# sirpkt/flink-tensorflow

Hardware: AMD Instinct MI355X
Metric: records/sec (whole node) + p50 per-record latency, ResNet-50 stream DP=1/8 (higher is better)
Workload: dtype bf16

## Files before the change

### flink_tensorflow_amd/kernels/conv_pp.hip

```cpp
#include <pybind11/pybind11.h>

#include <stdexcept>
#include <string>
#include <type_traits>

#include "common.h"

namespace {


struct CSrc {
  const bf16* x;
  int H, W, C;
  int sh, sw, ph, pw;
};

struct CPParams {
  CSrc s[2];
  const bf16* w;
  const float* bias;
  const bf16* res;
  void* y;
  int M, N, K;
  int OH, OW;
  int KW, dh, dw;
  int ldw, ldy, y_coff, ldr;
  int tiles_m, tiles_n;
  int nk0;
};

FTM_DEVICE int lite_slot(int row, int chunk) { return chunk ^ (row & 7); }

template <int ACT, bool HAS_RES, bool DUAL = false>
__global__ __launch_bounds__(256, 2) void conv_lite_kernel(CPParams p) {
  constexpr int BM = 128, BN = 128, BK = 64;
  constexpr int NT = 256;
  constexpr int ROWB = BK * 2;
  constexpr int RPI = 1024 / ROWB;
  constexpr int Q = 4;
  constexpr int NI = BN / 32;
  constexpr int PJ = 4;
  constexpr int XB = BM * ROWB, WB = BN * ROWB, STG = XB + WB;
  constexpr int OPITCH = BN * 2 + 16;
  constexpr int LDS = 2 * STG;
  static_assert(BM / RPI / 4 == Q && BN / RPI / 4 == Q && BM * OPITCH <= LDS, "tile geometry");
  __shared__ __attribute__((aligned(1024))) uint8_t smem[LDS];

  const int nwg = p.tiles_m * p.tiles_n;
  const int tile = xcd_remap(blockIdx.x, nwg);
  const int tm = tile / p.tiles_n;
  const int tn = tile - tm * p.tiles_n;
  const int m0 = tm * BM;
  const int n0 = tn * BN;
  const int lane = threadIdx.x & 63;
  const int wave = __builtin_amdgcn_readfirstlane(threadIdx.x >> 6);
  const int wm = wave & 1;
  const int wn = wave >> 1;

  const int drow = lane / 8;
  const int dchunk = lite_slot(drow, lane % 8);
  const unsigned nimg = (unsigned)p.M / (unsigned)(p.OH * p.OW);
  const CSrc& S = p.s[0];
  const __amdgpu_buffer_rsrc_t rx = __builtin_amdgcn_make_buffer_rsrc(
      (void*)S.x, 0, (int)(nimg * (unsigned)(S.H * S.W) * (unsigned)S.C * 2u), 0x00020000);
  const __amdgpu_buffer_rsrc_t rw = __builtin_amdgcn_make_buffer_rsrc(
      (void*)p.w, 0, (int)((unsigned)p.N * (unsigned)p.ldw * 2u), 0x00020000);
  int pb[4], hw[4], pb1[4];
  unsigned offw[4];
  const CSrc& S1 = p.s[1];
  __amdgpu_buffer_rsrc_t rx1 = rx;
  if constexpr (DUAL)
    rx1 = __builtin_amdgcn_make_buffer_rsrc((void*)S1.x, 0, (int)(nimg * (unsigned)(S1.H * S1.W) * (unsigned)S1.C * 2u),
                                            0x00020000);
  const int ohw = p.OH * p.OW;
#pragma unroll
  for (int q = 0; q < Q; ++q) {
    const unsigned co = n0 + RPI * (Q * wave + q) + drow;
    offw[q] = co < (unsigned)p.N ? (co * p.ldw + dchunk * 8) * 2u : 0x80000000u;
    const int r = RPI * (Q * wave + q) + drow;
    const int m = m0 + r;
    const bool live = m < p.M;
    const int n = live ? m / ohw : 0;
    const int rem = live ? m - n * ohw : 0;
    const int oh = rem / p.OW;
    const int ow = rem - oh * p.OW;
    const int ih0 = live ? oh * S.sh - S.ph : -16384;
    const int iw0 = ow * S.sw - S.pw;
    pb[q] = ((n * S.H + ih0) * S.W + iw0) * S.C * 2 + dchunk * 16;
    hw[q] = (ih0 << 16) | (iw0 & 0xFFFF);
    if constexpr (DUAL) pb1[q] = live ? ((n * S1.H + oh * S1.sh) * S1.W + ow * S1.sw) * S1.C * 2 + dchunk * 16 : -1;
  }
  const int cpt = S.C / BK;
  int cc = 0, kw = 0, kh = 0, kt_dma = 0;
  auto dma = [&](int stage) {
    const unsigned woff = (unsigned)kt_dma * (unsigned)ROWB;
    if constexpr (DUAL) {
      if (kt_dma >= p.nk0) {
        const int delta1 = (kt_dma - p.nk0) * BK * 2;
        ++kt_dma;
        uint8_t* bx = smem + stage * STG + Q * wave * RPI * ROWB;
        uint8_t* bw = smem + stage * STG + XB + Q * wave * RPI * ROWB;
#pragma unroll
        for (int q = 0; q < Q; ++q) {
          __builtin_amdgcn_raw_ptr_buffer_load_lds(rx1, (__attribute__((address_space(3))) void*)(bx + q * 1024), 16,
                                                   pb1[q] >= 0 ? (unsigned)(pb1[q] + delta1) : 0x80000000u, 0, 0, 0);
          __builtin_amdgcn_raw_ptr_buffer_load_lds(rw, (__attribute__((address_space(3))) void*)(bw + q * 1024), 16,
                                                   offw[q], woff, 0, 0);
        }
        return;
      }
    }
    const int dih = kh * p.dh, diw = kw * p.dw;
    const int delta = ((dih * S.W + diw) * S.C + cc * BK) * 2;
    ++kt_dma;
    if (++cc == cpt) {
      cc = 0;
      if (++kw == p.KW) {
        kw = 0;
        ++kh;
      }
    }
    uint8_t* bx = smem + stage * STG + Q * wave * RPI * ROWB;
    uint8_t* bw = smem + stage * STG + XB + Q * wave * RPI * ROWB;
#pragma unroll
    for (int q = 0; q < Q; ++q) {
      const int ih = (hw[q] >> 16) + dih;
      const int iw = ((hw[q] << 16) >> 16) + diw;
      const bool ok = (unsigned)ih < (unsigned)S.H && (unsigned)iw < (unsigned)S.W;
      __builtin_amdgcn_raw_ptr_buffer_load_lds(rx, (__attribute__((address_space(3))) void*)(bx + q * 1024), 16,
                                               ok ? (unsigned)(pb[q] + delta) : 0x80000000u, 0, 0, 0);
      __builtin_amdgcn_raw_ptr_buffer_load_lds(rw, (__attribute__((address_space(3))) void*)(bw + q * 1024), 16,
                                               offw[q], woff, 0, 0);
    }
  };

  const int frow = lane & 15;
  const int fq = lane >> 4;
  f32x4 acc[NI][PJ];
#pragma unroll
  for (int i = 0; i < NI; ++i)
#pragma unroll
    for (int j = 0; j < PJ; ++j) acc[i][j] = f32x4{0.f, 0.f, 0.f, 0.f};

  const int nk = p.K / BK;
  dma(0);
  for (int kt = 0; kt < nk; ++kt) {
    const int st = kt & 1;
    asm volatile("s_waitcnt vmcnt(0)" ::: "memory");
    __syncthreads();
    if (kt + 1 < nk) dma(st ^ 1);
    const uint8_t* xs = smem + st * STG;
    const uint8_t* ws = xs + XB;
    __builtin_amdgcn_s_setprio(1);
#pragma unroll
    for (int ks = 0; ks < BK / 32; ++ks) {
      const int sl = lite_slot(frow, ks * 4 + fq) << 4;
      bf16x8 a[NI], b[PJ];
#pragma unroll
      for (int i = 0; i < NI; ++i)
        a[i] = *reinterpret_cast<const bf16x8*>(ws + (wn * (BN / 2) + i * 16 + frow) * ROWB + sl);
#pragma unroll
      for (int j = 0; j < PJ; ++j) b[j] = *reinterpret_cast<const bf16x8*>(xs + (wm * 64 + j * 16 + frow) * ROWB + sl);
#pragma unroll
      for (int i = 0; i < NI; ++i)
#pragma unroll
        for (int j = 0; j < PJ; ++j) acc[i][j] = __builtin_amdgcn_mfma_f32_16x16x32_bf16(a[i], b[j], acc[i][j], 0, 0, 0);
    }
    __builtin_amdgcn_s_setprio(0);
  }
  __syncthreads();

#pragma unroll
  for (int i = 0; i < NI; ++i) {
    const int cl = wn * (BN / 2) + i * 16 + fq * 4;
    f32x4 bv = {0.f, 0.f, 0.f, 0.f};
    if (p.bias && n0 + cl < p.N) bv = *reinterpret_cast<const f32x4*>(p.bias + n0 + cl);
#pragma unroll
    for (int j = 0; j < PJ; ++j) {
      const int pl = wm * 64 + j * 16 + frow;
      bf16x4 o;
#pragma unroll
      for (int r = 0; r < 4; ++r) {
        float v = acc[i][j][r] + bv[r];
        if constexpr (!HAS_RES) v = apply_act<ACT>(v);
        o[r] = f2bf(v);
      }
      *reinterpret_cast<bf16x4*>(smem + pl * OPITCH + cl * 2) = o;
    }
  }
  __syncthreads();
  bf16* y = reinterpret_cast<bf16*>(p.y);
  constexpr int SEGS = BN / 8;
#pragma unroll 4
  for (int q = threadIdx.x; q < BM * SEGS; q += NT) {
    const int ml = q / SEGS;
    const int ccol = q - ml * SEGS;
    const int m = m0 + ml;
    const int n = n0 + ccol * 8;
    if (m >= p.M || n >= p.N) continue;
    u32x4 v = *reinterpret_cast<const u32x4*>(smem + ml * OPITCH + ccol * 16);
    if constexpr (HAS_RES) {
      bf16x8 o = __builtin_bit_cast(bf16x8, v);
      const bf16x8 r = *reinterpret_cast<const bf16x8*>(p.res + (size_t)m * p.ldr + n);
#pragma unroll
      for (int e = 0; e < 8; ++e) o[e] = f2bf(apply_act<ACT>((float)o[e] + (float)r[e]));
      v = __builtin_bit_cast(u32x4, o);
    }
    *reinterpret_cast<u32x4*>(y + (size_t)m * p.ldy + p.y_coff + n) = v;
  }
}

template <int ACT>
void launch_lite(const CPParams& p, hipStream_t s, bool dual) {
  const dim3 grid(p.tiles_m * p.tiles_n), block(256);
  if (dual) {
    if (p.res) hipLaunchKernelGGL((conv_lite_kernel<ACT, true, true>), grid, block, 0, s, p);
    else hipLaunchKernelGGL((conv_lite_kernel<ACT, false, true>), grid, block, 0, s, p);
    return;
  }
  if (p.res) hipLaunchKernelGGL((conv_lite_kernel<ACT, true>), grid, block, 0, s, p);
  else hipLaunchKernelGGL((conv_lite_kernel<ACT, false>), grid, block, 0, s, p);
}

void need(bool ok, const char* what) {
  if (!ok) throw std::invalid_argument(std::string("conv_pp: ") + what);
}

}

void conv_pp(pybind11::list srcs, uintptr_t w, uintptr_t bias, uintptr_t res, uintptr_t y, int N, int OH, int OW,
             int Cout, int ldy, int y_coff, int ldr, int act, uintptr_t stream) {
  const int ns = (int)pybind11::len(srcs);
  need(ns == 1 || ns == 2, "one or two sources");
  CPParams p{};
  long K = 0;
  for (int i = 0; i < ns; ++i) {
    pybind11::tuple t = srcs[i].cast<pybind11::tuple>();
    need(t.size() == 13, "source tuple (x, N, H, W, C, KH, KW, sh, sw, ph, pw, dh, dw)");
    CSrc& S = p.s[i];
    S.x = reinterpret_cast<const bf16*>(t[0].cast<uintptr_t>());
    const int n = t[1].cast<int>();
    S.H = t[2].cast<int>(); S.W = t[3].cast<int>(); S.C = t[4].cast<int>();
    const int KH = t[5].cast<int>(), KW = t[6].cast<int>();
    S.sh = t[7].cast<int>(); S.sw = t[8].cast<int>(); S.ph = t[9].cast<int>(); S.pw = t[10].cast<int>();
    const int dh = t[11].cast<int>(), dw = t[12].cast<int>();
    need(n == N, "source batch != output batch");
    need(S.C % 64 == 0, "input channels must be a multiple of 64");
    need(reinterpret_cast<uintptr_t>(S.x) % 16 == 0, "x alignment");
    need((long)N * S.H * S.W * S.C * 2 < (1L << 31), "input larger than 2 GiB");
    need(S.H < 16384 && S.W < 16384 && S.ph < 1024 && S.pw < 1024, "spatial size");
    need((KH - 1) * dh < 1024 && (KW - 1) * dw < 1024, "receptive field");
    K += (long)KH * KW * S.C;
    if (i == 0) {
      p.KW = KW;
      p.dh = dh;
      p.dw = dw;
      p.nk0 = (int)(K / 64);
    } else {
      need(KH == 1 && KW == 1 && S.ph == 0 && S.pw == 0, "the 4-wave tile's second source must be 1x1 unpadded");
      need((OH - 1) * S.sh < S.H && (OW - 1) * S.sw < S.W, "second source smaller than the output grid");
    }
  }
  for (int i = ns; i < 2; ++i) p.s[i] = p.s[0];
  need(Cout % 8 == 0 && ldy % 8 == 0 && y_coff % 8 == 0, "Cout / ldy / y_coff must be multiples of 8");
  need(!res || ldr % 8 == 0, "ldr alignment");
  need(w % 16 == 0 && y % 16 == 0 && (!bias || bias % 16 == 0) && (!res || res % 16 == 0), "alignment");
  need((long)Cout * K * 2 < (1L << 31), "weights larger than 2 GiB");
  p.w = reinterpret_cast<const bf16*>(w);
  p.bias = reinterpret_cast<const float*>(bias);
  p.res = reinterpret_cast<const bf16*>(res);
  p.y = reinterpret_cast<void*>(y);
  p.M = N * OH * OW;
  p.N = Cout;
  p.K = (int)K;
  p.OH = OH; p.OW = OW;
  p.ldw = (int)K; p.ldy = ldy; p.y_coff = y_coff; p.ldr = ldr;
  p.tiles_m = (p.M + 127) / 128;
  p.tiles_n = (Cout + 127) / 128;
  hipStream_t s = reinterpret_cast<hipStream_t>(stream);
  if (act == ACT_RELU) launch_lite<ACT_RELU>(p, s, ns == 2);
  else if (act == ACT_NONE) launch_lite<ACT_NONE>(p, s, ns == 2);
  else throw std::invalid_argument("conv_pp: unsupported activation");
  FTM_CHECK_LAUNCH();
}

void register_conv_pp(pybind11::module_& m) {
  m.def("conv_pp", &conv_pp);
}
```

### flink_tensorflow_amd/ops/kernels.py

```python
from __future__ import annotations

import copy
import functools
import math
import os

import torch
import torch.nn.functional as F

from .. import _ext

ACT_NONE, ACT_RELU, ACT_GELU, ACT_SIGMOID, ACT_TANH, ACT_RELU6, ACT_DRELU = 0, 1, 2, 3, 4, 5, 6
_ACT_NAMES = {None: ACT_NONE, "none": ACT_NONE, "relu": ACT_RELU, "gelu": ACT_GELU, "gelu_tanh": ACT_GELU,
              "sigmoid": ACT_SIGMOID, "tanh": ACT_TANH, "relu6": ACT_RELU6, "drelu": ACT_DRELU}


def act_code(act) -> int:
    if isinstance(act, int):
        return act
    try:
        return _ACT_NAMES[act]
    except KeyError:
        raise ValueError(f"unknown activation {act!r}") from None

# ... 182 lines not shown
    if tuple(w3.reshape(w3.shape[0], -1).shape) != (co, k3) or tuple(w1.reshape(cn, -1).shape) != (cn, co):
        raise ValueError(f"bottleneck_tail: weights must be [{co}, {k3}] and [{cn}, {co}], got {tuple(w3.shape)} "
                         f"{tuple(w1.shape)}")
    if b3.numel() != co or b1.numel() != cn:
        raise ValueError("bottleneck_tail: bias sizes must match the output channels")
    odt = x2.dtype if x2.is_cuda else torch.float32
    lead3 = (lead[0], dec_hw[0] // 2, dec_hw[1] // 2) if y3_decimated else lead
    y3 = torch.empty((*lead3, co), dtype=odt, device=x2.device) if y3 is None else y3
    y1 = torch.empty((*lead, cn), dtype=odt, device=x2.device) if y1 is None else y1
    if tuple(y3.shape) != (*lead3, co) or tuple(y1.shape) != (*lead, cn):
        raise ValueError("bottleneck_tail: output buffers do not fit")
    M = x2.numel() // cx
    second = xs if dual else res
    if x2.is_cuda:
        for t, n in ((x2, "x2"), (second, "xs" if dual else "res"), (w3, "w3"), (w1, "w1"), (y3, "y3"), (y1, "y1")):
            _check(t, n, device=x2.device)
        _check(b3, "b3", torch.float32, x2.device)
        _check(b1, "b1", torch.float32, x2.device)
        dev = x2.device.index if x2.device.index is not None else torch.cuda.current_device()
        _hip().bottleneck_tail_bf16(x2.data_ptr(), _ptr(xs), _ptr(res), w3.data_ptr(), b3.data_ptr(),
                                    w1.data_ptr(), b1.data_ptr(), y3.data_ptr(), y1.data_ptr(), M, cn,
                                    _NUM_CU[dev], _stream(), dec_hw[0], dec_hw[1])
        return y3, y1
    xin = torch.cat([x2.reshape(M, cx), xs.reshape(M, cx)], 1) if dual else x2.reshape(M, cx)
    a = xin.float() @ w3.reshape(co, k3).float().t() + b3.float()
    a = a.to(odt).float()
    a = torch.relu(a if dual else a + res.reshape(M, co).float()).to(y3.dtype)
    y3.copy_(a.reshape(*lead, co)[:, ::2, ::2] if y3_decimated else a.reshape(y3.shape))
    b = torch.relu(a.float() @ w1.reshape(cn, co).float().t() + b1.float())
    y1.copy_(b.reshape(y1.shape).to(y1.dtype))
    return y3, y1


def bottleneck_chain(links, w1: torch.Tensor, b1: torch.Tensor, y1: torch.Tensor | None = None,
                     y3: torch.Tensor | None = None, y3_decimated: bool = False, store_y3: bool = True):
    x0 = links[0][0]
    lead = x0.shape[:-1]
    M = x0.numel() // 64
    cn = w1.shape[0]
    if not 1 <= len(links) <= 3 or links[0][1] is None or any(l[1] is not None for l in links[1:]):
        raise ValueError("bottleneck_chain: 1 to 3 links, the first dual ([x | xs]), the others plain")
    for j, (x, xs, w, b) in enumerate(links):
        if x.shape[-1] != 64 or x.numel() != M * 64 or (xs is not None and tuple(xs.shape) != tuple(x.shape)):
            raise ValueError("bottleneck_chain: every source is [..., 64] over the same pixels")
        if tuple(w.reshape(w.shape[0], -1).shape) != (256, 128 if j == 0 else 64) or b.numel() != 256:
            raise ValueError(f"bottleneck_chain: link {j} weights must be [256, {128 if j == 0 else 64}]")
    if cn not in (64, 128) or tuple(w1.reshape(cn, -1).shape) != (cn, 256) or b1.numel() != cn:
        raise ValueError("bottleneck_chain: w1 must be [64 or 128, 256]")
    dec_hw = (0, 0)
    if y3_decimated:
        if x0.dim() != 4 or x0.shape[1] % 2 or x0.shape[2] % 2:
            raise ValueError("bottleneck_chain: decimated y3 needs [N, H, W, 64] sources with even H, W")
        dec_hw = (x0.shape[1], x0.shape[2])
    odt = x0.dtype if x0.is_cuda else torch.float32
    lead3 = (lead[0], dec_hw[0] // 2, dec_hw[1] // 2) if y3_decimated else lead
    if store_y3 and y3 is None:
        y3 = torch.empty((*lead3, 256), dtype=odt, device=x0.device)
    y1 = torch.empty((*lead, cn), dtype=odt, device=x0.device) if y1 is None else y1
    if (store_y3 and tuple(y3.shape) != (*lead3, 256)) or tuple(y1.shape) != (*lead, cn):
        raise ValueError("bottleneck_chain: output buffers do not fit")
    if x0.is_cuda:
        for j, (x, xs, w, b) in enumerate(links):
            for t, n in ((x, "x"), (w, "w")) + (((xs, "xs"),) if xs is not None else ()):
                _check(t, f"link {j} {n}", device=x0.device)
            _check(b, f"link {j} bias", torch.float32, x0.device)
        _check(w1, "w1", device=x0.device)
        _check(b1, "b1", torch.float32, x0.device)
        _check(y1, "y1", device=x0.device)
        if store_y3:
            _check(y3, "y3", device=x0.device)
        dev = x0.device.index if x0.device.index is not None else torch.cuda.current_device()
        _hip().bottleneck_chain_bf16([(x.data_ptr(), _ptr(xs), w.data_ptr(), b.data_ptr()) for x, xs, w, b in links],
                                     w1.data_ptr(), b1.data_ptr(), y3.data_ptr() if store_y3 else 0, y1.data_ptr(), M,
                                     cn, _NUM_CU[dev], _stream(), dec_hw[0], dec_hw[1])
        return (y3 if store_y3 else None), y1
    y = None
    rdt = y1.dtype
    for x, xs, w, b in links:
        xin = torch.cat([x.reshape(M, 64), xs.reshape(M, 64)], 1) if xs is not None else x.reshape(M, 64)
        a = (xin.float() @ w.reshape(256, -1).float().t() + b.float()).to(odt).float()
        y = torch.relu(a if y is None else a + y).to(rdt).float()
    if store_y3:
        y3.copy_(y.reshape(*lead, 256)[:, ::2, ::2] if y3_decimated else y.reshape(y3.shape))
    y1.copy_(torch.relu(y @ w1.reshape(cn, 256).float().t() + b1.float()).reshape(y1.shape).to(y1.dtype))
    return (y3 if store_y3 else None), y1


def gemm(x: torch.Tensor, w_nk: torch.Tensor, bias: torch.Tensor | None = None, residual: torch.Tensor | None = None,
         act=None, out: torch.Tensor | None = None, cfg: int = -1) -> torch.Tensor:
    a = act_code(act)
    lead = x.shape[:-1]
    K = x.shape[-1]
    N, K2 = w_nk.shape
    if K != K2:
        raise ValueError(f"gemm: K mismatch {K} vs {K2}")
    x2 = x.reshape(-1, K)
    M = x2.shape[0]
    if out is None:
        out = torch.empty((*lead, N), dtype=x.dtype if x.is_cuda else torch.float32, device=x.device)
    out2 = out.reshape(M, N)
    if residual is not None and residual.numel() != M * N:
        raise ValueError("gemm: residual shape mismatch")
    if x.is_cuda:
        _check(x2, "x", device=x.device)
        _check(w_nk, "w", device=x.device)
        _check(out2, "out", device=x.device)
        if bias is not None:
            _check(bias, "bias", torch.float32, x.device)
        else:
            bias = _zeros_bias(N, x.device)
        if residual is not None:
            _check(residual, "residual", device=x.device)
        _hip().gemm_bf16(x2.data_ptr(), w_nk.data_ptr(), bias.data_ptr(), _ptr(residual), out2.data_ptr(), M, N, K, K,
                         N, N, a, _stream(), cfg)
        return out
    y = x2.float() @ w_nk.float().t()
    if bias is not None:
        y = y + bias.float()
    if residual is not None:
        y = y + residual.reshape(M, N).float()
    out2.copy_(_apply_act_ref(y, a).to(out.dtype))
    return out


_TR_KTILE_US = 0.45
_TR_KTILE_DEEP_US = 0.3
_TR_SLOTS = 512


def _tr_time(tiles: int, per: int, se: int, num_cu: int = 256) -> float:
    wgs = tiles * se
    if wgs <= num_cu:
        return per * _TR_KTILE_DEEP_US
    return -(-wgs // _TR_SLOTS) * per * _TR_KTILE_US


def gemm_train_splits(M: int, N: int, K: int) -> int:
    tiles = -(-M // 128) * -(-N // 128)
    nk = -(-K // 64)
    best_s, best_t = 1, _tr_time(tiles, nk, 1)
    for s in (2, 3, 4, 6, 8, 12, 16, 24, 32):
        if s > nk:
            break
        per = -(-nk // s)
        se = -(-nk // per)
        t = _tr_time(tiles, per, se) + se * M * N * 8 / _PP_SPLIT_BW + 2.0
        if t < 0.9 * best_t:
            best_s, best_t = se, t
    return best_s


def gemm_train(x: torch.Tensor, w: torch.Tensor, *, x_t: bool = False, w_t: bool = False,
               bias: torch.Tensor | None = None, mask: torch.Tensor | None = None, act=None,
               out: torch.Tensor | None = None, out_dtype=torch.bfloat16, splits: int | None = None,
               ws: torch.Tensor | None = None, colsum: torch.Tensor | None = None) -> torch.Tensor:
    a = act_code(act)
    if mask is not None:
        if a not in (ACT_NONE, ACT_DRELU):
            raise ValueError("gemm_train: mask is the ReLU-backward operand; it takes no other activation")
        a = ACT_DRELU
    M, K = (x.shape[1], x.shape[0]) if x_t else (x.shape[0], x.shape[1])
    N, K2 = (w.shape[1], w.shape[0]) if w_t else (w.shape[0], w.shape[1])
    if K != K2:
        raise ValueError(f"gemm_train: K mismatch {K} vs {K2}")
    if out is None:
        out = torch.empty((M, N), dtype=out_dtype, device=x.device)
    if tuple(out.shape) != (M, N):
        raise ValueError(f"gemm_train: out shape {tuple(out.shape)} != {(M, N)}")
    f32 = out.dtype == torch.float32
    if not x.is_cuda:
        X = x.float().t() if x_t else x.float()
        W = w.float() if w_t else w.float().t()
        y = X @ W
        if bias is not None:
            y = y + bias.float()
        if mask is not None:
            y = torch.where(mask.float() > 0, y, torch.zeros_like(y))
        else:
            y = _apply_act_ref(y, a)
        out.copy_(y.to(out.dtype))
        if colsum is not None:
            yq = out.float()
            for t in range(colsum.shape[0]):
                colsum[t].copy_(yq[t * 128:(t + 1) * 128].sum(0))
        return out
    for t, nm in ((x, "x"), (w, "w")):
        if t.dtype != torch.bfloat16 or t.device != x.device or t.dim() != 2 or t.stride(1) != 1:
            raise ValueError(f"gemm_train: {nm} must be a bf16 [rows, cols] view with contiguous rows on {x.device}")
    if out.stride(1) != 1:
        raise ValueError("gemm_train: out rows must be contiguous")
    if bias is not None:
        _check(bias, "bias", torch.float32, x.device)
    if mask is not None:
        if mask.dtype != torch.bfloat16 or mask.device != x.device:
            raise ValueError(f"gemm_train: mask must be bf16 on {x.device}")
        if tuple(mask.shape) != (M, N) or mask.stride(1) != 1:
            raise ValueError("gemm_train: mask must be [M, N] with contiguous rows")
    if colsum is not None:
        if f32 or tuple(colsum.shape) != (-(-M // 128), N) or colsum.dtype != torch.float32 or not colsum.is_contiguous():
            raise ValueError("gemm_train: colsum must be contiguous fp32 [ceil(M/128), N] with bf16 output")
        splits = 1
    s = gemm_train_splits(M, N, K) if splits is None else int(splits)
    s = _hip().gemm_train_splits(K, s)
    wsp = 0
    if s > 1:
        need = s * M * N
        if ws is None or ws.numel() < need:
            ws = torch.empty(need, dtype=torch.float32, device=x.device)
        wsp = ws.data_ptr()
    _hip().gemm_train(x.data_ptr(), w.data_ptr(), _ptr(bias), _ptr(mask), out.data_ptr(), M, N, K, x.stride(0),
                      w.stride(0), out.stride(0), mask.stride(0) if mask is not None else 0, bool(x_t), bool(w_t), a,
                      f32, s, wsp, _ptr(colsum), _stream())
    return out


def colsum_reduce(part: torch.Tensor, out: torch.Tensor) -> torch.Tensor:
    T, N = part.shape
    if out.numel() != N:
        raise ValueError("colsum_reduce: out must hold N floats")
    if not part.is_cuda:
        out.copy_(part.sum(0).reshape(out.shape))
        return out
    if part.stride(1) != 1 or not out.is_contiguous():
        raise ValueError("colsum_reduce: contiguous rows / output")
    _hip().colsum_reduce(part.data_ptr(), T, part.stride(0), N, out.data_ptr(), _stream())
    return out


_PP_KTILE_US = 1.5
_PP_SPLIT_BW = 5.0e6


def gemm_pp_splits(M: int, N: int, K: int, num_cu: int = 256) -> int:
    tiles = -(-M // 256) * -(-N // 256)
    nk = K // 64
    best_s, best_t = 1, -(-tiles // num_cu) * nk * _PP_KTILE_US
    for s in range(2, min(16, nk) + 1):
        per = -(-nk // s)
        se = -(-nk // per)
        t = -(-tiles * se // num_cu) * per * _PP_KTILE_US + 2.0 * se * M * N * 4 / _PP_SPLIT_BW + 2.0
        if t < 0.9 * best_t:
            best_s, best_t = se, t
    return best_s


def gemm_pp(x: torch.Tensor, w_nk: torch.Tensor, bias: torch.Tensor | None = None,
            residual: torch.Tensor | None = None, act=None, out: torch.Tensor | None = None,
            splits: int | None = None, out_col: int = 0, ws: torch.Tensor | None = None) -> torch.Tensor:
    a = act_code(act)
    lead = x.shape[:-1]
    K = x.shape[-1]
    N, K2 = w_nk.shape
    if K != K2:
        raise ValueError(f"gemm_pp: K mismatch {K} vs {K2}")
    x2 = x.reshape(-1, K)
    M = x2.shape[0]
    if out is None:
        out = torch.empty((*lead, N), dtype=x.dtype if x.is_cuda else torch.float32, device=x.device)
    ldy = out.shape[-1]
    out2 = out.reshape(-1, ldy)
    if out2.shape[0] != M or out_col + N > ldy:
        raise ValueError("gemm_pp: output shape mismatch")
    if residual is not None and residual.numel() != M * N:
        raise ValueError("gemm_pp: residual shape mismatch")
    if x.is_cuda:
        if K % 64 or N % 8 or ldy % 8 or out_col % 8:
            raise ValueError("gemm_pp: needs K % 64 == 0 and N, ldy, out_col % 8 == 0")
        _check(x2, "x", device=x.device)
        _check(w_nk, "w", device=x.device)
        _check(out2, "out", device=x.device)
        if bias is not None:
            _check(bias, "bias", torch.float32, x.device)
        if residual is not None:
            _check(residual, "residual", device=x.device)
        if splits is None:
            splits = gemm_pp_splits(M, N, K)
        splits = _hip().gemm_pp_splits(K, splits)
        if splits > 1:
            if ws is None:
                ws = torch.empty(splits * M * N, dtype=torch.float32, device=x.device)
            elif ws.dtype != torch.float32 or ws.device != x.device or ws.numel() < splits * M * N:
                raise ValueError(f"gemm_pp: workspace needs {splits * M * N} fp32 elements on {x.device}")
        else:
            ws = None
        _hip().gemm_pp(x2.data_ptr(), w_nk.data_ptr(), _ptr(bias), _ptr(residual), out2.data_ptr(), M, N, K, K, K,
                       ldy, out_col, N, a, splits, _ptr(ws), _stream())
        return out
    y = x2.float() @ w_nk.float().t()
    if bias is not None:
        y = y + bias.float()
    if a == ACT_DRELU:
        if residual is None:
            raise ValueError("gemm_pp: act 'drelu' needs the mask operand (residual)")
        out2[:, out_col:out_col + N] = torch.where(residual.reshape(M, N).float() > 0, y, 0.0).to(out.dtype)
        return out
    if residual is not None:
        y = y + residual.reshape(M, N).float()
    out2[:, out_col:out_col + N] = _apply_act_ref(y, a).to(out.dtype)
    return out


class ConvPP:

    def __init__(self, srcs, Cout: int, out_hw, device, tile: None = None, splits: None = None):
        if tile is not None or splits is not None:
            raise TypeError("conv_pp: the tile and splits arguments are gone (one tile, no split-K)")
        self.srcs = [(tuple(xs), tuple(k), tuple(st), tuple(pd), tuple(dl)) for xs, k, st, pd, dl in srcs]
        self.N = self.srcs[0][0][0]
        self.OH, self.OW = out_hw
        self.Cout = Cout
        self.K = sum(k[0] * k[1] * xs[3] for xs, k, _, _, _ in self.srcs)
        for xs, _, _, _, _ in self.srcs:
            if xs[3] % 64 or xs[0] != self.N:
                raise ValueError("conv_pp: channels must be multiples of 64 and batches equal")
        if Cout % 8:
            raise ValueError("conv_pp: Cout % 8")
        self.M = self.N * self.OH * self.OW
        if len(self.srcs) == 2:
            (xs1, k1, st1, pd1, dl1) = self.srcs[1]
            if tuple(k1) != (1, 1) or tuple(pd1) != (0, 0) or (self.OH - 1) * st1[0] >= xs1[1] \
                    or (self.OW - 1) * st1[1] >= xs1[2]:
                raise ValueError("conv_pp: the 4-wave tile's second source must be 1x1, unpadded, in range")

    def for_batch(self, n: int) -> "ConvPP":
        if n == self.N:
            return self
        subs = self.__dict__.setdefault("_subs", {})
        sub = subs.get(n)
        if sub is None:
            sub = copy.copy(self)
            sub.srcs = [((n, *xs[1:]), k, st, pd, dl) for xs, k, st, pd, dl in self.srcs]
            sub.N, sub.M, sub._subs = n, n * self.OH * self.OW, {}
            if n > self.N:
                raise ValueError("conv_pp: a batch slice larger than the planned batch")
            subs[n] = sub
        return sub

    def __call__(self, xs, w, bias=None, residual=None, act=None, out=None, out_channel_offset: int = 0):
        if len(xs) != len(self.srcs):
            raise ValueError("conv_pp: source count")
        if xs and xs[0].dim() == 4 and xs[0].shape[0] != self.N:
            return self.for_batch(int(xs[0].shape[0]))(xs, w, bias, residual, act, out, out_channel_offset)
        for x, (shape, *_r) in zip(xs, self.srcs):
            if tuple(x.shape) != shape:
                raise ValueError(f"conv_pp: input shape {tuple(x.shape)} != planned {shape}")
        if out is None:
            out = torch.empty((self.N, self.OH, self.OW, self.Cout), dtype=torch.bfloat16, device=xs[0].device)
        ldy = out.shape[-1]
        if tuple(out.shape[:3]) != (self.N, self.OH, self.OW) or out_channel_offset + self.Cout > ldy:
            raise ValueError("conv_pp: output shape mismatch")
        if tuple(w.shape) != (self.Cout, self.K):
            raise ValueError(f"conv_pp: weight {tuple(w.shape)} != ({self.Cout}, {self.K})")
        if not xs[0].is_cuda:
            return self._reference(xs, w, bias, residual, act, out, out_channel_offset)
        for i, x in enumerate(xs):
            _check(x, f"x{i}", device=out.device)
        _check(w, "w", device=out.device)
        _check(out, "out", device=out.device)
        if bias is not None:
            _check(bias, "bias", torch.float32, out.device)
        if residual is not None:
            _check(residual, "residual", device=out.device)
            if residual.numel() != self.M * self.Cout:
                raise ValueError("conv_pp: residual shape")
        srcs = [(x.data_ptr(), self.N, sh[1], sh[2], sh[3], k[0], k[1], st[0], st[1], pd[0], pd[1], dl[0], dl[1])
                for x, (sh, k, st, pd, dl) in zip(xs, self.srcs)]
        _hip().conv_pp(srcs, w.data_ptr(), _ptr(bias), _ptr(residual), out.data_ptr(), self.N, self.OH, self.OW,
                       self.Cout, ldy, out_channel_offset, self.Cout, act_code(act), _stream())
        return out

    def _reference(self, xs, w, bias, residual, act, out, coff):
        import torch.nn.functional as F

        y = 0
        k0 = 0
        for x, (sh, (KH, KW), (s_h, s_w), (pt, pl), (dh, dw)) in zip(xs, self.srcs):
            C = sh[3]
            wk = w[:, k0:k0 + KH * KW * C].float().reshape(self.Cout, KH, KW, C).permute(0, 3, 1, 2)
            k0 += KH * KW * C
            xi = x.float().permute(0, 3, 1, 2)
            ph_hi = max(0, (self.OH - 1) * s_h + (KH - 1) * dh + 1 - sh[1] - pt)
            pw_hi = max(0, (self.OW - 1) * s_w + (KW - 1) * dw + 1 - sh[2] - pl)
            xi = F.pad(xi, (pl, pw_hi, pt, ph_hi))
            yi = F.conv2d(xi, wk, stride=(s_h, s_w), dilation=(dh, dw))[:, :, :self.OH, :self.OW]
            y = y + yi
        y = y.permute(0, 2, 3, 1)
        if bias is not None:
            y = y + bias.float()
        if residual is not None:
            y = y + residual.reshape(y.shape).float()
        out[..., coff:coff + self.Cout] = _apply_act_ref(y, act_code(act)).to(out.dtype)
        return out


def preprocess_images(images_u8: torch.Tensor, out_hw=(224, 224), mean=(117.0, 117.0, 117.0),
                      std=(1.0, 1.0, 1.0), align_corners=False, half_pixel_centers=False,
                      out: torch.Tensor | None = None, s2d: bool = False) -> torch.Tensor:
    if images_u8.dtype != torch.uint8 or images_u8.dim() != 4 or images_u8.shape[3] != 3:
        raise ValueError("preprocess_images expects uint8 [B,H,W,3]")
    B, Hi, Wi, _ = images_u8.shape
    Ho, Wo = out_hw
    oshape = (B, (Ho + 1) // 2, (Wo + 1) // 2, 16) if s2d else (B, Ho, Wo, 8)
    if out is None:
        out = torch.empty(oshape, dtype=torch.bfloat16 if images_u8.is_cuda else torch.float32,
                          device=images_u8.device)
    if tuple(out.shape) != oshape:
        raise ValueError(f"preprocess_images: out must be {oshape}, got {tuple(out.shape)}")
    if images_u8.is_cuda:
        if not images_u8.is_contiguous():
            raise ValueError("preprocess_images: input must be contiguous")
        _check(out, "out", device=images_u8.device)
        _hip().preprocess_u8_to_bf16(images_u8.data_ptr(), out.data_ptr(), B, Hi, Wi, Ho, Wo, int(align_corners),
                                     int(half_pixel_centers), float(mean[0]), float(mean[1]), float(mean[2]),
                                     1.0 / std[0], 1.0 / std[1], 1.0 / std[2], Hi * Wi * 3, int(s2d), _stream())
        return out
    from ..graph.ops_nn import resize_bilinear_tf

    y = resize_bilinear_tf(images_u8.float(), Ho, Wo, align_corners, half_pixel_centers)
    y = (y - torch.tensor(mean)) / torch.tensor(std)
    out.zero_()
    if s2d:
        Hb, Wb = (Ho + 1) // 2, (Wo + 1) // 2
        y = F.pad(y, (0, 0, 0, 2 * Wb - Wo, 0, 2 * Hb - Ho))
        blk = y.reshape(B, Hb, 2, Wb, 2, 3).permute(0, 1, 3, 2, 4, 5).reshape(B, Hb, Wb, 12)
        out[..., :12] = blk.to(out.dtype)
    else:
        out[..., :3] = y.to(out.dtype)
    return out


def jpeg_idct_rgb(coef: torch.Tensor, headers: torch.Tensor, out: torch.Tensor, n: int, H: int, W: int,
                  stream: int | None = None, threads: int = 8) -> torch.Tensor:
    if out.dtype != torch.uint8 or out.dim() != 4 or tuple(out.shape[1:]) != (H, W, 3) or not out.is_contiguous():
        raise ValueError(f"jpeg_idct_rgb: out must be contiguous uint8 [n, {H}, {W}, 3]")
    if coef.dim() != 2 or headers.dim() != 2 or not coef.is_contiguous() or not headers.is_contiguous():
        raise ValueError("jpeg_idct_rgb: coef and headers are contiguous [n, row bytes]")
    if n < 0 or n > min(coef.shape[0], headers.shape[0], out.shape[0]):
        raise ValueError("jpeg_idct_rgb: n exceeds the rows given")
    if coef.device != out.device or headers.device != out.device:
        raise ValueError("jpeg_idct_rgb: coef, headers and out must be on one device")
    stride = coef.shape[1] * coef.element_size()
    hbytes = headers.shape[1] * headers.element_size()
    if hbytes != _ext.native().jpeg_coeff_layout(H, W)[1]:
        raise ValueError("jpeg_idct_rgb: headers are not jpeg_coeff_layout's size")
    if out.is_cuda:
        _hip().jpeg_idct_rgb(coef.data_ptr(), headers.data_ptr(), out.data_ptr(), n, H, W, stride,
                             _stream() if stream is None else stream)
    else:
        _ext.native().jpeg_coeffs_to_rgb(coef.data_ptr(), n * stride, headers.data_ptr(), n * hbytes, out.data_ptr(),
                                         n * H * W * 3, n, stride, H * W * 3, H, W, threads)
    return out


def s2d_stem_weights(w_hwio: torch.Tensor, H: int, W: int, pads):
    KH, KW, C, Cout = w_hwio.shape
    pt, pb, pl, pr = pads
    if C != 3 or pt % 2 or pl % 2:
        raise ValueError("s2d stem needs RGB input and even top/left padding")
    KBH, KBW = (KH + 1) // 2, (KW + 1) // 2
    w2 = torch.zeros(Cout, KBH, KBW, 16, dtype=torch.float32)
    wf = w_hwio.float()
    for kh in range(KH):
        for kw in range(KW):
            ch = ((kh % 2) * 2 + (kw % 2)) * 3
            w2[:, kh // 2, kw // 2, ch:ch + 3] = wf[kh, kw].t()
    Ho = (H + pt + pb - KH) // 2 + 1
    Wo = (W + pl + pr - KW) // 2 + 1
    Hb, Wb = (H + 1) // 2, (W + 1) // 2
    pt_b, pl_b = pt // 2, pl // 2
    pb_b = Ho - 1 + KBH - Hb - pt_b
    pr_b = Wo - 1 + KBW - Wb - pl_b
    if pb_b < 0 or pr_b < 0:
        raise ValueError("s2d stem: negative block padding")
    return w2, (pt_b, pb_b, pl_b, pr_b)


DWCONV_TILES = {"1x4": 1, "2x2": 2}
DWCONV_GENERIC = -1


def dwconv_eligible(C: int, KH: int, KW: int, stride=(1, 1), dilation=(1, 1)) -> bool:
    return (C > 0 and C % 8 == 0 and 1 <= KH <= 7 and 1 <= KW <= 7 and min(stride) >= 1 and min(dilation) >= 1)


def dwconv_impl(KH: int, KW: int, stride=(1, 1), dilation=(1, 1)) -> str:
    if (KH, KW) == (3, 3) and tuple(dilation) == (1, 1) and tuple(stride) in ((1, 1), (2, 2)):
        return "dwconv3x3"
    return "dwconv_generic"


def dwconv2d_nhwc(x: torch.Tensor, w_taps_c: torch.Tensor, bias: torch.Tensor | None = None, stride=(1, 1),
                  pad=(0, 0, 0, 0), dilation=(1, 1), act=None, out: torch.Tensor | None = None,
                  out_channel_offset: int = 0, kernel=None, tile: int = 0) -> torch.Tensor:
    a = act_code(act)
    if a not in (ACT_NONE, ACT_RELU, ACT_RELU6):
        raise ValueError("dwconv2d_nhwc: act must be none, relu or relu6")
    N, H, W, C = x.shape
    taps, C2 = w_taps_c.shape
    if kernel is None:
        k = int(round(taps ** 0.5))
        kernel = (k, k)
    KH, KW = kernel
    if KH * KW != taps or C2 != C:
        raise ValueError(f"dwconv2d_nhwc: weights {tuple(w_taps_c.shape)} do not match a {KH}x{KW} filter over {C} "
                         f"channels")
    sh, sw = stride
    pt, pb, pl, pr = pad
    dh, dw = dilation
    if not dwconv_eligible(C, KH, KW, stride, dilation) or min(pad) < 0:
        raise ValueError(f"dwconv2d_nhwc: unsupported C={C}, {KH}x{KW}, stride {stride}, dilation {dilation}, "
                         f"pad {pad}")
    Ho, Wo = conv_out_hw(H, W, KH, KW, sh, sw, pt, pl, dh, dw, pb, pr)
    if Ho < 1 or Wo < 1:
        raise ValueError("dwconv2d_nhwc: empty output")
    if out is None:
        out = torch.empty((N, Ho, Wo, C), dtype=x.dtype if x.is_cuda else torch.float32, device=x.device)
        out_channel_offset = 0
    if out.dim() != 4 or out.shape[:3] != (N, Ho, Wo) or out_channel_offset < 0 \
            or out_channel_offset + C > out.shape[3]:
        raise ValueError(f"dwconv2d_nhwc: out {tuple(out.shape)} cannot hold [{N},{Ho},{Wo},{C}] at "
                         f"offset {out_channel_offset}")
    if x.is_cuda:
        for t, n in ((x, "x"), (w_taps_c, "w"), (out, "out")):
            _check(t, n, device=x.device)
        if bias is not None:
            _check(bias, "bias", torch.float32, x.device)
            if bias.numel() != C:
                raise ValueError("dwconv2d_nhwc: bias must have C elements")
        if out.shape[3] % 8 or out_channel_offset % 8:
            raise ValueError("dwconv2d_nhwc: output row pitch and channel offset must be multiples of 8")
        _hip().dwconv_nhwc_bf16(x.data_ptr(), w_taps_c.data_ptr(), _ptr(bias), out.data_ptr(), N, H, W, C, Ho, Wo,
                                KH, KW, sh, sw, dh, dw, pt, pl, a, out.shape[3], out_channel_offset, tile, _stream())
        return out
    xn = F.pad(x.float().permute(0, 3, 1, 2), (pl, pr, pt, pb))
    wn = w_taps_c.float().reshape(KH, KW, C).permute(2, 0, 1).unsqueeze(1)
    y = F.conv2d(xn, wn, stride=(sh, sw), dilation=(dh, dw), groups=C)
    if bias is not None:
        y = y + bias.float().view(1, -1, 1, 1)
    y = _apply_act_ref(y, a)
    out[..., out_channel_offset:out_channel_offset + C] = y.permute(0, 2, 3, 1).to(out.dtype)
    return out


DECONV_TILES = {"128x128": 0, "256x64": 1}


def deconv_eligible(Cin: int, Cout: int, KH: int, KW: int, stride=(2, 2)) -> bool:
    return (Cin > 0 and Cin % 8 == 0 and Cout > 0 and Cout % 8 == 0 and 1 <= KH <= 8 and 1 <= KW <= 8
            and len(stride) == 2 and all(1 <= s <= 4 for s in stride))


def _deconv_pads(pad) -> tuple[int, int]:
    return (int(pad[0]), int(pad[2])) if len(pad) == 4 else (int(pad[0]), int(pad[1]))


def deconv_phases(kernel, stride, pad, Cin: int = 1, Cout: int = 1) -> list[dict]:
    (KH, KW), (sh, sw), (pt, pl) = kernel, stride, _deconv_pads(pad)
    out, off = [], 0
    for py in range(sh):
        for px in range(sw):
            taps = [(ky, kx, (py + pt - ky) // sh, (px + pl - kx) // sw)
                    for ky in range(KH) if (py + pt - ky) % sh == 0
                    for kx in range(KW) if (px + pl - kx) % sw == 0]
            out.append({"py": py, "px": px, "taps": taps, "k": len(taps) * Cin, "offset": off})
            off += len(taps) * Cin * Cout
    return out


def deconv_pack_weights(w: torch.Tensor, stride, pad) -> torch.Tensor:
    KH, KW, Cout, Cin = w.shape
    parts = []
    for ph in deconv_phases((KH, KW), stride, pad, Cin, Cout):
        if ph["taps"]:
            parts.append(torch.stack([w[ky, kx] for ky, kx, _, _ in ph["taps"]], dim=1).reshape(-1))
    return torch.cat(parts).contiguous()


def deconv_unpack_weights(w_packed: torch.Tensor, kernel, stride, pad, Cin: int, Cout: int) -> torch.Tensor:
    KH, KW = kernel
    w = torch.zeros((KH, KW, Cout, Cin), dtype=w_packed.dtype, device=w_packed.device)
    for ph in deconv_phases(kernel, stride, pad, Cin, Cout):
        m = w_packed[ph["offset"]:ph["offset"] + Cout * ph["k"]].reshape(Cout, len(ph["taps"]), Cin)
        for t, (ky, kx, _, _) in enumerate(ph["taps"]):
            w[ky, kx] = m[:, t]
    return w


def deconv2d_nhwc(x: torch.Tensor, w_packed: torch.Tensor, bias: torch.Tensor | None, out_hw, kernel, stride=(2, 2),
                  pad=(0, 0, 0, 0), act=None, out: torch.Tensor | None = None, out_channel_offset: int = 0,
                  cfg: int = -1) -> torch.Tensor:
    a = act_code(act)
    if a not in (ACT_NONE, ACT_RELU, ACT_RELU6):
        raise ValueError("deconv2d_nhwc: act must be none, relu or relu6")
    if x.dim() != 4 or w_packed.dim() != 1:
        raise ValueError("deconv2d_nhwc: x must be [N, Hi, Wi, Cin] and w_packed flat")
    N, Hi, Wi, Cin = x.shape
    (KH, KW), (sh, sw), (Ho, Wo) = (int(v) for v in kernel), (int(v) for v in stride), (int(v) for v in out_hw)
    pt, pl = _deconv_pads(pad)
    taps = KH * KW
    if min(N, Hi, Wi, Cin, taps) < 1 or w_packed.numel() % (taps * Cin) or w_packed.numel() == 0:
        raise ValueError(f"deconv2d_nhwc: {w_packed.numel()} packed weights do not match a {KH}x{KW} filter over "
                         f"{Cin} input channels")
    Cout = w_packed.numel() // (taps * Cin)
    if not deconv_eligible(Cin, Cout, KH, KW, (sh, sw)) or not (0 <= pt < KH and 0 <= pl < KW):
        raise ValueError(f"deconv2d_nhwc: unsupported Cin={Cin}, Cout={Cout}, {KH}x{KW}, stride {(sh, sw)}, "
                         f"pad {(pt, pl)}")
    if Ho < 1 or Wo < 1:
        raise ValueError("deconv2d_nhwc: empty output")
    if cfg not in (-1, *DECONV_TILES.values()):
        raise ValueError(f"deconv2d_nhwc: unknown tile configuration {cfg}")
    if out is None:
        out = torch.empty((N, Ho, Wo, Cout), dtype=x.dtype if x.is_cuda else torch.float32, device=x.device)
        out_channel_offset = 0
    if out.dim() != 4 or out.shape[:3] != (N, Ho, Wo) or out_channel_offset < 0 \
            or out_channel_offset + Cout > out.shape[3]:
        raise ValueError(f"deconv2d_nhwc: out {tuple(out.shape)} cannot hold [{N},{Ho},{Wo},{Cout}] at "
                         f"offset {out_channel_offset}")
    if bias is not None and bias.numel() != Cout:
        raise ValueError("deconv2d_nhwc: bias must have Cout elements")
    if x.is_cuda:
        for t, n in ((x, "x"), (w_packed, "w_packed"), (out, "out")):
            _check(t, n, device=x.device)
        if bias is not None:
            _check(bias, "bias", torch.float32, x.device)
        else:
            bias = _zeros_bias(Cout, x.device)
        if out.shape[3] % 8 or out_channel_offset % 8:
            raise ValueError("deconv2d_nhwc: output row pitch and channel offset must be multiples of 8")
        _hip().deconv_nhwc_bf16(x.data_ptr(), w_packed.data_ptr(), bias.data_ptr(), out.data_ptr(), N, Hi, Wi, Cin,
                                Ho, Wo, Cout, KH, KW, sh, sw, pt, pl, a, out.shape[3], out_channel_offset,
                                w_packed.numel(), cfg, _stream())
        return out
    xf = x.float()
    y = torch.zeros((N, Ho, Wo, Cout), dtype=torch.float32)
    for ph in deconv_phases((KH, KW), (sh, sw), (pt, pl), Cin, Cout):
        sub = y[:, ph["py"]::sh, ph["px"]::sw]
        Hq, Wq = sub.shape[1:3]
        m = w_packed[ph["offset"]:ph["offset"] + Cout * ph["k"]].float().reshape(Cout, len(ph["taps"]), Cin)
        for t, (_, _, dy, dx) in enumerate(ph["taps"]):
            q0, q1 = max(0, -dy), min(Hq, Hi - dy)
            r0, r1 = max(0, -dx), min(Wq, Wi - dx)
            if q0 < q1 and r0 < r1:
                sub[:, q0:q1, r0:r1] += xf[:, q0 + dy:q1 + dy, r0 + dx:r1 + dx] @ m[:, t].t()
    if bias is not None:
        y = y + bias.float()
    y = _apply_act_ref(y, a)
    out[..., out_channel_offset:out_channel_offset + Cout] = y.to(out.dtype)
    return out


CONV3D_TILES = {"128x128": 0, "256x64": 1}


def conv3d_eligible(Cin: int, Cout: int, kernel, stride, dilation=(1, 1, 1)) -> bool:
    return (Cin > 0 and Cin % 8 == 0 and Cout > 0 and Cout % 8 == 0 and len(kernel) == 3 and len(stride) == 3
            and all(1 <= k <= 7 for k in kernel) and all(1 <= s <= 4 for s in stride) and tuple(dilation) == (1, 1, 1))


def conv3d_pack_weights(w: torch.Tensor) -> torch.Tensor:
    KD, KH, KW, Cin, Cout = w.shape
    return w.permute(4, 0, 1, 2, 3).reshape(Cout, KD * KH * KW * Cin).contiguous()


def conv3d_unpack_weights(w_packed: torch.Tensor, kernel, Cin: int) -> torch.Tensor:
    KD, KH, KW = kernel
    return w_packed.reshape(w_packed.shape[0], KD, KH, KW, Cin).permute(1, 2, 3, 4, 0).contiguous()


def _out3d(name: str, ext, k, s, pad):
    if len(pad) != 6 or min(pad) < 0:
        raise ValueError(f"{name}: pad must be six non-negative values (front, back, top, bottom, left, right)")
# ... 1059 lines not shown
```

Baseline: 81940.

## Add persistent conv kernel with cross-tile DMA prefetch and buffer-resource loads

Adds a persistent variant of the implicit-GEMM conv kernel. It launches at most two workgroups per CU, loops over tiles, and prefetches the next tile's first K-slice and bias while the current tile finishes, so the prologue overlaps the previous epilogue. It uses buffer resources for out-of-bounds-safe loads and stores, and it stages the epilogue through LDS. The path is picked automatically when there are at least twice as many tiles as slots, and callers now pass the CU count. The cost is more complex synchronisation and new 2 GiB limits on output and residual.

New measurement: 81800. No clear change (-0.2%).

```diff
diff --git a/flink_tensorflow_amd/kernels/conv_pp.hip b/flink_tensorflow_amd/kernels/conv_pp.hip
--- a/flink_tensorflow_amd/kernels/conv_pp.hip
+++ b/flink_tensorflow_amd/kernels/conv_pp.hip
@@ -8,6 +8,8 @@
 
 namespace {
 
+
+typedef uint32_t u32x2 __attribute__((ext_vector_type(2)));
 
 struct CSrc {
   const bf16* x;
@@ -210,6 +212,264 @@
   }
 }
 
+template <int ACT, bool HAS_RES, bool DUAL = false>
+__global__ __launch_bounds__(256, 2) void conv_lite_persistent_kernel(CPParams p) {
+  constexpr int BM = 128, BN = 128, BK = 64;
+  constexpr int ROWB = BK * 2;
+  constexpr int RPI = 1024 / ROWB;
+  constexpr int Q = 4;
+  constexpr int NI = BN / 32;
+  constexpr int PJ = 4;
+  constexpr int XB = BM * ROWB, WB = BN * ROWB, STG = XB + WB;
+  constexpr int LDS = 2 * STG;
+  constexpr unsigned OOB = 0x80000000u;
+  __shared__ __attribute__((aligned(1024))) uint8_t smem[LDS];
+
+  const int nwg = p.tiles_m * p.tiles_n, tiles_n = p.tiles_n;
+  const int G = gridDim.x, b0 = blockIdx.x;
+  const int M = p.M, N = p.N, OW = p.OW, ohw = p.OH * p.OW, ldw = p.ldw;
+  const unsigned ldy = p.ldy, y_coff = p.y_coff, ldr = p.ldr;
+  const int nk = p.K / BK, nk0 = p.nk0, KW = p.KW, dh = p.dh, dw = p.dw;
+  const CSrc S = p.s[0], S1 = p.s[1];
+  const int lane = threadIdx.x & 63;
+  const int wave = __builtin_amdgcn_readfirstlane(threadIdx.x >> 6);
+  const int wm = wave & 1;
+  const int wn = wave >> 1;
+  const int drow = lane / 8;
+  const int dchunk = lite_slot(drow, lane % 8);
+  const int frow = lane & 15;
+  const int fq = lane >> 4;
+
+  const unsigned nimg = (unsigned)M / (unsigned)ohw;
+  const __amdgpu_buffer_rsrc_t rx = __builtin_amdgcn_make_buffer_rsrc(
+      (void*)S.x, 0, (int)(nimg * (unsigned)(S.H * S.W) * (unsigned)S.C * 2u), 0x00020000);
+  const __amdgpu_buffer_rsrc_t rw =
+      __builtin_amdgcn_make_buffer_rsrc((void*)p.w, 0, (int)((unsigned)N * (unsigned)ldw * 2u), 0x00020000);
+  __amdgpu_buffer_rsrc_t rx1 = rx;
+  if constexpr (DUAL)
+    rx1 = __builtin_amdgcn_make_buffer_rsrc((void*)S1.x, 0, (int)(nimg * (unsigned)(S1.H * S1.W) * (unsigned)S1.C * 2u),
+                                            0x00020000);
+  const __amdgpu_buffer_rsrc_t ry =
+      __builtin_amdgcn_make_buffer_rsrc(p.y, 0, (int)((unsigned)M * ldy * 2u), 0x00020000);
+  const __amdgpu_buffer_rsrc_t rb =
+      __builtin_amdgcn_make_buffer_rsrc((void*)p.bias, 0, p.bias ? N * 4 : 0, 0x00020000);
+  const __amdgpu_buffer_rsrc_t rr = __builtin_amdgcn_make_buffer_rsrc(
+      (void*)p.res, 0, HAS_RES ? (int)((unsigned)M * ldr * 2u) : 0, 0x00020000);
+
+  int pb[4], hw[4], pb1[4], dn0 = 0;
+  unsigned offw[4];
+  float bln = 0.f;
+  auto origins = [&](int v) {
+    const int tile = xcd_remap(v, nwg);
+    const int tm = tile / tiles_n;
+    const int m0 = tm * BM, n0 = (tile - tm * tiles_n) * BN;
+    dn0 = n0;
+#pragma unroll
+    for (int q = 0; q < Q; ++q) {
+      const unsigned co = n0 + RPI * (Q * wave + q) + drow;
+      offw[q] = co < (unsigned)N ? (co * ldw + dchunk * 8) * 2u : OOB;
+      const unsigned m = m0 + RPI * (Q * wave + q) + drow;
+      const bool live = m < (unsigned)M;
+      const unsigned n = live ? m / (unsigned)ohw : 0;
+      const unsigned rem = live ? m - n * ohw : 0;
+      const int oh = rem / (unsigned)OW;
+      const int ow = rem - oh * OW;
+      const int ih0 = live ? oh * S.sh - S.ph : -16384;
+      const int iw0 = ow * S.sw - S.pw;
+      pb[q] = (((int)n * S.H + ih0) * S.W + iw0) * S.C * 2 + dchunk * 16;
+      hw[q] = (ih0 << 16) | (iw0 & 0xFFFF);
+      if constexpr (DUAL)
+        pb1[q] = live ? (((int)n * S1.H + oh * S1.sh) * S1.W + ow * S1.sw) * S1.C * 2 + dchunk * 16 : -1;
+    }
+  };
+  const int cpt = S.C / BK;
+  int cc = 0, kw = 0, kh = 0, kt_dma = 0;
+  auto dma = [&](int stage) {
+    const unsigned woff = (unsigned)kt_dma * (unsigned)ROWB;
+    uint8_t* bx = smem + stage * STG + Q * wave * RPI * ROWB;
+    uint8_t* bw = bx + XB;
+    if constexpr (DUAL) {
+      if (kt_dma >= nk0) {
+        const int delta1 = (kt_dma - nk0) * BK * 2;
+        ++kt_dma;
+#pragma unroll
+        for (int q = 0; q < Q; ++q) {
+          __builtin_amdgcn_raw_ptr_buffer_load_lds(rx1, (__attribute__((address_space(3))) void*)(bx + q * 1024), 16,
+                                                   pb1[q] >= 0 ? (unsigned)(pb1[q] + delta1) : OOB, 0, 0, 0);
+          __builtin_amdgcn_raw_ptr_buffer_load_lds(rw, (__attribute__((address_space(3))) void*)(bw + q * 1024), 16,
+                                                   offw[q], woff, 0, 0);
+        }
+        return;
+      }
+    }
+    const int dih = kh * dh, diw = kw * dw;
+    const int delta = ((dih * S.W + diw) * S.C + cc * BK) * 2;
+    ++kt_dma;
+    if (++cc == cpt) {
+      cc = 0;
+      if (++kw == KW) {
+        kw = 0;
+        ++kh;
+      }
+    }
+#pragma unroll
+    for (int q = 0; q < Q; ++q) {
+      const int ih = (hw[q] >> 16) + dih;
+      const int iw = ((hw[q] << 16) >> 16) + diw;
+      const bool ok = (unsigned)ih < (unsigned)S.H && (unsigned)iw < (unsigned)S.W;
+      __builtin_amdgcn_raw_ptr_buffer_load_lds(rx, (__attribute__((address_space(3))) void*)(bx + q * 1024), 16,
+                                               ok ? (unsigned)(pb[q] + delta) : OOB, 0, 0, 0);
+      __builtin_amdgcn_raw_ptr_buffer_load_lds(rw, (__attribute__((address_space(3))) void*)(bw + q * 1024), 16,
+                                               offw[q], woff, 0, 0);
+    }
+  };
+  auto load_bias = [&]() {
+    bln = __builtin_bit_cast(float, __builtin_amdgcn_raw_buffer_load_b32(rb, (dn0 + wn * 64 + lane) * 4, 0, 0));
+  };
+  int vd = b0;
+  auto wrap = [&]() {
+    if (kt_dma < nk) return false;
+    kt_dma = cc = kw = kh = 0;
+    vd += G;
+    return vd < nwg;
+  };
+
+  origins(vd);
+  load_bias();
+  dma(0);
+  asm volatile("" : "+v"(bln));
+  if (wrap()) origins(vd);
+  int st = 0;
+
+  for (int vc = b0; vc < nwg; vc += G) {
+    const int tile = xcd_remap(vc, nwg);
+    const int tm = tile / tiles_n;
+    const int m0 = tm * BM, n0 = (tile - tm * tiles_n) * BN;
+    f32x4 acc[NI][PJ];
+#pragma unroll
+    for (int i = 0; i < NI; ++i)
+#pragma unroll
+      for (int j = 0; j < PJ; ++j) acc[i][j] = f32x4{0.f, 0.f, 0.f, 0.f};
+    float bl = 0.f;
+
+    for (int kt = 0; kt < nk; ++kt) {
+      if (kt == 0 && vc != b0) {
+        asm volatile("s_waitcnt vmcnt(8) lgkmcnt(0)" ::: "memory");
+      } else {
+        asm volatile("s_waitcnt vmcnt(0) lgkmcnt(0)" ::: "memory");
+      }
+      __builtin_amdgcn_s_barrier();
+      if (kt == 0) {
+        asm volatile("" : "+v"(bln));
+        bl = bln;
+      }
+      bool fresh = false;
+      if (vd < nwg) {
+        if (kt_dma == 0) load_bias();
+        dma(st ^ 1);
+        fresh = wrap();
+      }
+      const uint8_t* xs = smem + st * STG;
+      const uint8_t* ws = xs + XB;
+      __builtin_amdgcn_s_setprio(1);
+#pragma unroll
+      for (int ks = 0; ks < BK / 32; ++ks) {
+        const int sl = lite_slot(frow, ks * 4 + fq) << 4;
+        bf16x8 a[NI], b[PJ];
+#pragma unroll
+        for (int i = 0; i < NI; ++i)
+          a[i] = *reinterpret_cast<const bf16x8*>(ws + (wn * (BN / 2) + i * 16 + frow) * ROWB + sl);
+#pragma unroll
+        for (int j = 0; j < PJ; ++j) b[j] = *reinterpret_cast<const bf16x8*>(xs + (wm * 64 + j * 16 + frow) * ROWB + sl);
+#pragma unroll
+        for (int i = 0; i < NI; ++i)
+#pragma unroll
+          for (int j = 0; j < PJ; ++j) acc[i][j] = __builtin_amdgcn_mfma_f32_16x16x32_bf16(a[i], b[j], acc[i][j], 0, 0, 0);
+      }
+      __builtin_amdgcn_s_setprio(0);
+      st ^= 1;
+      if (fresh) origins(vd);
+    }
+
+    int efrow = frow, efq = fq, elane = lane;
+    asm volatile("" : "+v"(efrow), "+v"(efq), "+v"(elane));
+    const int erow = elane >> 3, echunk = elane & 7;
+    const unsigned en = n0 + wn * (BN / 2) + echunk * 8;
+    u32x4 rv[8];
+    if constexpr (HAS_RES) {
+#pragma unroll
+      for (int it = 0; it < 8; ++it) {
+        const unsigned m = m0 + wm * 64 + it * 8 + erow;
+        rv[it] = __builtin_bit_cast(u32x4, __builtin_amdgcn_raw_buffer_load_b128(
+                                               rr, m < (unsigned)M && en < (unsigned)N ? (m * ldr + en) * 2u : OOB, 0, 0));
+      }
+    }
+    asm volatile("s_waitcnt lgkmcnt(0)" ::: "memory");
+    __builtin_amdgcn_s_barrier();
+    uint8_t* ot = smem + (st ^ 1) * STG + wave * (64 * ROWB);
+#pragma unroll
+    for (int i = 0; i < NI; ++i) {
+      bf16x4 o[PJ];
+#pragma unroll
+      for (int r = 0; r < 4; ++r) {
+        const float bv = __builtin_bit_cast(
+            float, __builtin_amdgcn_ds_bpermute((i * 16 + efq * 4 + r) * 4, __builtin_bit_cast(int, bl)));
+#pragma unroll
+        for (int j = 0; j < PJ; ++j) {
+          float v = acc[i][j][r] + bv;
+          if constexpr (!HAS_RES) v = apply_act<ACT>(v);
+          o[j][r] = f2bf(v);
+        }
+      }
+#pragma unroll
+      for (int j = 0; j < PJ; ++j) {
+        const int row = j * 16 + efrow;
+        *reinterpret_cast<bf16x4*>(ot + row * ROWB + (lite_slot(row, i * 2 + (efq >> 1)) << 4) + (efq & 1) * 8) = o[j];
+      }
+    }
+#pragma unroll
+    for (int it = 0; it < 8; ++it) {
+      const int row = it * 8 + erow;
+      const unsigned m = m0 + wm * 64 + row;
+      u32x4 v = *reinterpret_cast<const u32x4*>(ot + row * ROWB + (lite_slot(row, echunk) << 4));
+      if constexpr (HAS_RES) {
+        bf16x8 o = __builtin_bit_cast(bf16x8, v);
+        const bf16x8 r = __builtin_bit_cast(bf16x8, rv[it]);
+#pragma unroll
+        for (int e = 0; e < 8; ++e) o[e] = f2bf(apply_act<ACT>((float)o[e] + (float)r[e]));
+        v = __builtin_bit_cast(u32x4, o);
+      }
+      __builtin_amdgcn_raw_buffer_store_b128(v, ry, m < (unsigned)M && en < (unsigned)N ? (m * ldy + y_coff + en) * 2u : OOB,
+                                             0, 0);
+    }
+  }
+}
+
+struct LiteShape {
+  bool persistent;
+  int grid;
+};
+LiteShape lite_shape(int tiles, int num_cu, int persistent, int max_wg) {
+  const int slots = 2 * num_cu;
+  const bool pers = persistent < 0 ? tiles >= 2 * slots : persistent != 0;
+  if (!pers) return {false, tiles};
+  int grid = tiles < slots ? tiles : slots;
+  if (max_wg > 0 && max_wg < grid) grid = max_wg;
+  return {true, grid};
+}
+
+template <int ACT>
+void launch_lite_persistent(const CPParams& p, hipStream_t s, bool dual, int wgs) {
+  const dim3 grid(wgs), block(256);
+  if (dual) {
+    if (p.res) hipLaunchKernelGGL((conv_lite_persistent_kernel<ACT, true, true>), grid, block, 0, s, p);
+    else hipLaunchKernelGGL((conv_lite_persistent_kernel<ACT, false, true>), grid, block, 0, s, p);
+    return;
+  }
+  if (p.res) hipLaunchKernelGGL((conv_lite_persistent_kernel<ACT, true>), grid, block, 0, s, p);
+  else hipLaunchKernelGGL((conv_lite_persistent_kernel<ACT, false>), grid, block, 0, s, p);
+}
+
 template <int ACT>
 void launch_lite(const CPParams& p, hipStream_t s, bool dual) {
   const dim3 grid(p.tiles_m * p.tiles_n), block(256);
@@ -229,7 +489,7 @@
 }
 
 void conv_pp(pybind11::list srcs, uintptr_t w, uintptr_t bias, uintptr_t res, uintptr_t y, int N, int OH, int OW,
-             int Cout, int ldy, int y_coff, int ldr, int act, uintptr_t stream) {
+             int Cout, int ldy, int y_coff, int ldr, int act, uintptr_t stream, int num_cu, int persistent, int max_wg) {
   const int ns = (int)pybind11::len(srcs);
   need(ns == 1 || ns == 2, "one or two sources");
   CPParams p{};
@@ -278,12 +538,27 @@
   p.tiles_m = (p.M + 127) / 128;
   p.tiles_n = (Cout + 127) / 128;
   hipStream_t s = reinterpret_cast<hipStream_t>(stream);
-  if (act == ACT_RELU) launch_lite<ACT_RELU>(p, s, ns == 2);
+  need(num_cu > 0, "num_cu");
+  const bool fits = (long)p.M * ldy * 2 < (1L << 31) && (!res || (long)p.M * ldr * 2 < (1L << 31));
+  need(fits || persistent <= 0, "persistent: output or residual larger than 2 GiB");
+  const LiteShape ls = lite_shape(p.tiles_m * p.tiles_n, num_cu, fits ? persistent : 0, max_wg);
+  if (ls.persistent) {
+    if (act == ACT_RELU) launch_lite_persistent<ACT_RELU>(p, s, ns == 2, ls.grid);
+    else if (act == ACT_NONE) launch_lite_persistent<ACT_NONE>(p, s, ns == 2, ls.grid);
+    else throw std::invalid_argument("conv_pp: unsupported activation");
+  } else if (act == ACT_RELU) launch_lite<ACT_RELU>(p, s, ns == 2);
   else if (act == ACT_NONE) launch_lite<ACT_NONE>(p, s, ns == 2);
   else throw std::invalid_argument("conv_pp: unsupported activation");
   FTM_CHECK_LAUNCH();
 }
 
+pybind11::tuple conv_pp_shape(int tiles, int num_cu, int persistent, int max_wg) {
+  need(tiles > 0 && num_cu > 0, "tiles / num_cu");
+  const LiteShape ls = lite_shape(tiles, num_cu, persistent, max_wg);
+  return pybind11::make_tuple(ls.persistent, ls.grid);
+}
+
 void register_conv_pp(pybind11::module_& m) {
   m.def("conv_pp", &conv_pp);
-}
+  m.def("conv_pp_shape", &conv_pp_shape);
+}
diff --git a/flink_tensorflow_amd/ops/kernels.py b/flink_tensorflow_amd/ops/kernels.py
--- a/flink_tensorflow_amd/ops/kernels.py
+++ b/flink_tensorflow_amd/ops/kernels.py
@@ -508,9 +508,14 @@
 
 class ConvPP:
 
-    def __init__(self, srcs, Cout: int, out_hw, device, tile: None = None, splits: None = None):
+    def __init__(self, srcs, Cout: int, out_hw, device, tile: None = None, splits: None = None,
+                 persistent: bool | None = None, max_workgroups: int | None = None):
         if tile is not None or splits is not None:
             raise TypeError("conv_pp: the tile and splits arguments are gone (one tile, no split-K)")
+        if max_workgroups is not None and max_workgroups < 1:
+            raise ValueError("conv_pp: max_workgroups < 1")
+        self.persistent = persistent
+        self.max_workgroups = max_workgroups
         self.srcs = [(tuple(xs), tuple(k), tuple(st), tuple(pd), tuple(dl)) for xs, k, st, pd, dl in srcs]
         self.N = self.srcs[0][0][0]
         self.OH, self.OW = out_hw
@@ -527,6 +532,16 @@
             if tuple(k1) != (1, 1) or tuple(pd1) != (0, 0) or (self.OH - 1) * st1[0] >= xs1[1] \
                     or (self.OW - 1) * st1[1] >= xs1[2]:
                 raise ValueError("conv_pp: the 4-wave tile's second source must be 1x1, unpadded, in range")
+
+    @property
+    def tiles(self) -> int:
+        return -(-self.M // 128) * -(-self.Cout // 128)
+
+    def launch_shape(self, num_cu: int) -> tuple[bool, int]:
+        return tuple(_hip().conv_pp_shape(self.tiles, num_cu, *self._path_args()))
+
+    def _path_args(self) -> tuple[int, int]:
+        return (-1 if self.persistent is None else int(bool(self.persistent)), self.max_workgroups or 0)
 
     def for_batch(self, n: int) -> "ConvPP":
         if n == self.N:
@@ -571,8 +586,10 @@
                 raise ValueError("conv_pp: residual shape")
         srcs = [(x.data_ptr(), self.N, sh[1], sh[2], sh[3], k[0], k[1], st[0], st[1], pd[0], pd[1], dl[0], dl[1])
                 for x, (sh, k, st, pd, dl) in zip(xs, self.srcs)]
+        dev = out.device.index if out.device.index is not None else torch.cuda.current_device()
         _hip().conv_pp(srcs, w.data_ptr(), _ptr(bias), _ptr(residual), out.data_ptr(), self.N, self.OH, self.OW,
-                       self.Cout, ldy, out_channel_offset, self.Cout, act_code(act), _stream())
+                       self.Cout, ldy, out_channel_offset, self.Cout, act_code(act), _stream(),
+                       _NUM_CU[dev], *self._path_args())
         return out
 
     def _reference(self, xs, w, bias, residual, act, out, coff):
```
